# anacarsi/ss25_Hierarchical_Multiscale_Image_Classification

Measured on AMD Instinct MI355X. Metric: 224x224 patches/sec (ResNet18 fwd), higher is better.
Workload: dtype bf16; 1 GPU; resnet18_fwd_880k_patches_bf16; input=uint8 HWC patches resident in HBM, outputs=features[B,512] + logits[B,2] + labels, weights=seeded random init, parallelism=single GPU

## Files before the change

ss25_hierarchical_multiscale_image_classification_amd/csrc/block16_c64.h:

```cpp
#pragma once
#include "halo16.h"

namespace hipac {

typedef __attribute__((ext_vector_type(2))) short s16x2;
__device__ __forceinline__ unsigned relu_pk(unsigned v) {
  return __builtin_bit_cast(unsigned, __builtin_elementwise_max(__builtin_bit_cast(s16x2, v), s16x2{0, 0}));
}

constexpr int kBlkRing = 30;
constexpr int kBlkXPitch = 18 * 128;
constexpr int kBlkIPitch = 16 * 128;
constexpr int kBlkXBytes = 32 * kBlkXPitch + 512;
constexpr int kBlkIBytes = 32 * kBlkIPitch + 256;
constexpr int kBlkRsBytes = 2 * 6144 + 2 * 4096;

#ifndef HIPAC_BLK16_AHEAD
#define HIPAC_BLK16_AHEAD 1
#endif

template <typename T, int NP, int PITCH>
__device__ __forceinline__ void c64_strip16_mfma(const typename Elem<T>::frag (&wreg)[9][2][2], const int (&lb)[NP][3],
                                                 const float* __restrict__ bl, f32x4 (&acc)[2 * NP][2]) {
  using frag = typename Elem<T>::frag;
  constexpr int NR = 2 * NP;
#pragma unroll
  for (int t = 0; t < 2; ++t) {
    const f32x4 b = *reinterpret_cast<const f32x4*>(bl + 16 * t);
#pragma unroll
    for (int i = 0; i < NR; ++i) acc[i][t] = b;
  }
  asm volatile("s_waitcnt lgkmcnt(0)" ::: "memory");
  constexpr int AH = HIPAC_BLK16_AHEAD;
  frag fr[AH + 1][NR];
  auto rd = [&](auto S, auto I) {
    constexpr int s = decltype(S)::value, i = decltype(I)::value;
    constexpr int tap = s >> 1, kk = s & 1, kh = tap / 3, kw = tap % 3;
    lds_read16<((i & 1) + kh) * PITCH>(fr[s % (AH + 1)][i], (unsigned)(lb[i >> 1][kw] ^ (kk << 6)));
  };
  __builtin_amdgcn_s_setprio(1);
  static_for<AH>([&](auto S) { static_for<NR>([&](auto I) { rd(S, I); }); });
  static_for<18>([&](auto S) {
    constexpr int s = decltype(S)::value, tap = s >> 1, kk = s & 1;
    static_for<NR>([&](auto I) {
      constexpr int i = decltype(I)::value;
      if constexpr (s + AH < 18) rd(std::integral_constant<int, s + AH>{}, I);
      constexpr int full = (18 - 1 - s < AH - 1 ? 18 - 1 - s : AH - 1);
      wait_lgkmcnt<(NR - 1 - i) + full * NR + (s + AH < 18 ? i + 1 : 0)>();
      Asm16<T>::mfma(acc[i][0], wreg[tap][kk][0], fr[s % (AH + 1)][i]);
      Asm16<T>::mfma(acc[i][1], wreg[tap][kk][1], fr[s % (AH + 1)][i]);
    });
  });
  __builtin_amdgcn_s_setprio(0);
  asm volatile("s_nop 7\n\ts_nop 7\n\ts_nop 3" ::: "memory");
}

template <typename T>
__global__ __launch_bounds__(512, 2) void block16_c64_kernel(const T* __restrict__ in, const T* __restrict__ w1,
                                                             const float* __restrict__ b1, const T* __restrict__ w2,
                                                             const float* __restrict__ b2, T* __restrict__ out,
                                                             int n_img) {
  using E = Elem<T>;
  using frag = typename E::frag;
  using vec4 = typename E::vec4;
  constexpr int H = 56, W = 56, C = 64, RING = kBlkRing, XP = kBlkXPitch, IP = kBlkIPitch;
  __shared__ __attribute__((aligned(1024))) unsigned char smem[kBlkXBytes + kBlkIBytes + kBlkRsBytes + 512];
  unsigned char* const Xr = smem;
  unsigned char* const Ir = smem + kBlkXBytes;
  float* const Bl = reinterpret_cast<float*>(smem + kBlkXBytes + kBlkIBytes + kBlkRsBytes);

  const int tid = threadIdx.x, lane = tid & 63;
  const int wave = __builtin_amdgcn_readfirstlane(tid >> 6);
  const int team = wave >> 2, tw = wave & 3, nh = tw & 1, mh = tw >> 1;
  const int n16 = lane & 15, g = lane >> 4;
  const int lx = n16 < 4 ? 2 * n16 : (n16 < 12 ? 2 * n16 - 7 : 2 * n16 - 16);
  unsigned char* const Rw = smem + kBlkXBytes + kBlkIBytes + (mh == 0 ? nh * 6144 : 2 * 6144 + nh * 4096);

  if (tid < 64) Bl[tid] = b1[tid];
  else if (tid < 128) Bl[tid] = b2[tid - 64];

  const int xcd = blockIdx.x & 7, slot = blockIdx.x >> 3, nslots = gridDim.x >> 3;
  const int n_x = n_img > xcd ? (n_img - xcd + 7) >> 3 : 0;
  const int nst = 4 * n_x;
  const int ns = nst > slot ? (nst - slot + nslots - 1) / nslots : 0;
  if (ns == 0) return;

  frag wreg[9][2][2];
  {
    const char* wb = reinterpret_cast<const char*>(team ? w2 : w1) + (size_t)(nh * 32 + n16) * (9 * C * 2) + 16 * g;
#pragma unroll
    for (int tap = 0; tap < 9; ++tap)
#pragma unroll
      for (int kk = 0; kk < 2; ++kk)
#pragma unroll
        for (int t = 0; t < 2; ++t) wreg[tap][kk][t] = *reinterpret_cast<const frag*>(wb + t * 16 * (9 * C * 2) + tap * 128 + kk * 64);
  }

  const rsrc_t x_rsrc = make_rsrc(in, n_img * (H * W * C * 2));

  constexpr int NKP = 5;
  int relo[NKP];
#pragma unroll
  for (int kp = 0; kp < NKP; ++kp) {
    const int q = 8 * (tw + 4 * kp) + (lane >> 3);
    const int rr = (q * 3641) >> 16;
    const int j = q - 18 * rr;
    const int c = (lane & 7) ^ ((j >> 1) & 7);
    relo[kp] = (((rr * W + j) << 7) + (c << 4)) | (j < 2 ? 1 : 0) | (j >= 16 ? 2 : 0) | (rr == 0 ? 4 : 0) | (rr >= 1 ? 8 : 0);
  }
  auto x_rows = [&](int img, int x0, int L0, int rb, int np, int rowmask) {
    const int sb = ((img * H + L0 - 1) * W + x0 - 2) << 7;
    const int smask = (x0 == 0 ? 1 : 0) | (x0 == 42 ? 2 : 0) | rowmask;
    static_for<NKP>([&](auto KP) {
      constexpr int kp = decltype(KP)::value;
      const int p = tw + 4 * kp;
      if (p < np) {
        asm volatile("" : "+v"(relo[kp]));
        const int off = (relo[kp] & smask) ? (int)0x80000000 : (relo[kp] & ~15) + sb;
        buffer_load_lds16(x_rsrc, Xr + rb * XP + p * 1024, off, 0);
      }
    });
  };
  auto x_group = [&](int img, int x0, int gq) {
    const int rb = 8 * gq >= RING ? 8 * gq - RING : 8 * gq;
    x_rows(img, x0, 8 * gq, rb, gq == 7 ? 5 : 18, gq == 0 ? 4 : (gq == 7 ? 8 : 0));
    if (gq == 3) x_rows(img, x0, RING, 0, 5, 0);
  };
  auto strip_img = [&](int k) { return (((slot + k * nslots) >> 2) << 3) + xcd; };
  auto strip_x0 = [&](int k) { return ((slot + k * nslots) & 3) * 14; };

  const int lds_base = (int)(unsigned)(size_t)(__attribute__((address_space(3))) unsigned char*)smem;
  int la[3];
#pragma unroll
  for (int kw = 0; kw < 3; ++kw) {
    const int j = lx + kw;
    la[kw] = (j << 7) + (((((j >> 1) & 7)) ^ g) << 4) + (team ? kBlkXBytes : 0) + lds_base;
  }
  const int iw_lane = (lx << 7) + ((g & 1) << 3);
  const int iw_pos = ((nh << 2) + (g >> 1)) ^ ((lx >> 1) & 7);
  const float* const bl = Bl + team * 64 + nh * 32 + 4 * g;

#pragma unroll
  for (int tap = 0; tap < 9; ++tap)
#pragma unroll
    for (int kk = 0; kk < 2; ++kk)
#pragma unroll
      for (int t = 0; t < 2; ++t) asm volatile("" ::"v"(wreg[tap][kk][t]));
  if (team == 0) {
    x_group(strip_img(0), strip_x0(0), 0);
    x_group(strip_img(0), strip_x0(0), 1);
    wait_vmcnt<0>();
  }
  asm volatile("s_waitcnt lgkmcnt(0)" ::: "memory");
  __builtin_amdgcn_s_barrier();

  const int n_steps = 7 * ns;
  f32x4 acc[4][2];
  int pend_n = 0, pend_y = 0;
  const int rs_px = lane >> 2;
  const int rs_off = (((rs_px < 14 ? rs_px : 13)) * C + nh * 32 + 8 * ((lane & 3) ^ ((rs_px >> 2) & 3))) * 2;
  auto fetch_resid = [&](int pix0, int y0, int sl) {
    const int sb = (pix0 + y0 * W) << 7;
#pragma unroll
    for (int rho = 0; rho < 2; ++rho) buffer_load_lds16(x_rsrc, Rw + sl * 2048 + rho * 1024, rs_off + rho * (W * C * 2), sb);
  };
  const int rs_rd = lx * 64 + 8 * (g & 1);
  const int rs_sw = (lx >> 2) & 3;
  const int out_lane = (lx * C + nh * 32 + 16 * (g & 1) + 8 * (g >> 1)) * 2;
  auto epilogue_b = [&](auto A0, int pix0, int y0, int sl) {
    constexpr int a0 = decltype(A0)::value;
#pragma unroll
    for (int rho = 0; rho < 2; ++rho) {
      unsigned P[2][2];
#pragma unroll
      for (int t = 0; t < 2; ++t) {
        const vec4 rv = *reinterpret_cast<const vec4*>(Rw + sl * 2048 + rho * 1024 + rs_rd + (((2 * t + (g >> 1)) ^ rs_sw) << 4));
        const f32x4& a = acc[a0 + rho][t];
        P[t][0] = relu_pk(PackPair<T>::pack_rn(a[0] + (float)rv[0], a[1] + (float)rv[1]));
        P[t][1] = relu_pk(PackPair<T>::pack_rn(a[2] + (float)rv[2], a[3] + (float)rv[3]));
      }
      permlane16_swap(P[0][0], P[1][0]);
      permlane16_swap(P[0][1], P[1][1]);
      char* const dst = reinterpret_cast<char*>(out) + ((size_t)(unsigned)(pix0 + (y0 + rho) * W) << 7) + out_lane;
      if (lx < 14) store16_out(dst, u32x4{P[0][0], P[0][1], P[1][0], P[1][1]});
    }
  };
  int pend_pix = 0, pend_sl = 0;
  auto flush_b = [&]() {
    if (pend_n) {
      wait_vmcnt<0>();
      epilogue_b(std::integral_constant<int, 0>{}, pend_pix, pend_y, pend_sl);
      if (pend_n == 2) epilogue_b(std::integral_constant<int, 2>{}, pend_pix, pend_y + 2, pend_sl + 1);
      pend_n = 0;
    }
  };
  auto step_barrier = [&]() {
    asm volatile("s_waitcnt lgkmcnt(0)" ::: "memory");
    __builtin_amdgcn_s_barrier();
  };
  if (team == 0) {
    for (int G = 0; G <= n_steps; ++G) {
      if (G < n_steps) {
        const int k = G / 7, m = G - 7 * k;
        const int img = strip_img(k), x0 = strip_x0(k);
        if (m <= 4) x_group(img, x0, m + 2);
        else if (m == 5) {
          x_group(img, x0, 7);
          if (k + 1 < ns) x_group(strip_img(k + 1), strip_x0(k + 1), 0);
        } else if (k + 1 < ns) x_group(strip_img(k + 1), strip_x0(k + 1), 1);
        if (m == 0 || m == 6)
          *reinterpret_cast<u32x2*>(Ir + (m == 0 ? 0 : 27) * IP + tw * 512 + lane * 8) = u32x2{0u, 0u};
        const int y0a = 8 * m + 4 * mh;
        int lb[2][3];
#pragma unroll
        for (int p = 0; p < 2; ++p) {
          const int y0 = y0a + 2 * p;
          const int wbase = (y0 >= RING ? y0 - RING : y0) * XP;
#pragma unroll
          for (int kw = 0; kw < 3; ++kw) lb[p][kw] = la[kw] + wbase;
        }
        c64_strip16_mfma<T, 2, XP>(wreg, lb, bl, acc);
        const bool col_ok = !((x0 == 0 && lx == 0) || (x0 == 42 && lx == 15));
#pragma unroll
        for (int i = 0; i < 4; ++i) {
          const int Lr = y0a + i + 1;
          const bool twice = Lr == RING || Lr == RING + 1;
          unsigned char* const dst = Ir + (Lr >= RING ? Lr - RING : Lr) * IP + iw_lane;
          unsigned char* const dst2 = Ir + Lr * IP + iw_lane;
#pragma unroll
          for (int t = 0; t < 2; ++t) {
            u32x2 pk;
            pk[0] = relu_pk(PackPair<T>::pack_rn(acc[i][t][0], acc[i][t][1]));
            pk[1] = relu_pk(PackPair<T>::pack_rn(acc[i][t][2], acc[i][t][3]));
            if (!col_ok) pk = u32x2{0u, 0u};
            *reinterpret_cast<u32x2*>(dst + ((iw_pos ^ (2 * t)) << 4)) = pk;
            if (twice) *reinterpret_cast<u32x2*>(dst2 + ((iw_pos ^ (2 * t)) << 4)) = pk;
          }
        }
      }
      wait_vmcnt<0>();
      step_barrier();
    }
  } else {
    for (int G = 0; G <= n_steps; ++G) {
      flush_b();
      if (G >= 1) {
        const int k = (G - 1) / 7, mp = G - 7 * k;
        int yp = 8 * mp - 10 + 4 * mh, ys = -1;
        bool has_pair = true;
        if (mp == 1) {
          if (mh == 0) yp = 0;
          else has_pair = false, ys = 4;
        } else if (mp == 7) {
          if (mh == 0) yp = 46, ys = 50;
          else yp = 52;
        }
        const int pix0 = strip_img(k) * (H * W) + strip_x0(k);
        if (has_pair) {
          fetch_resid(pix0, yp, 0);
          fetch_resid(pix0, yp + 2, 1);
        }
        if (ys >= 0) fetch_resid(pix0, ys, has_pair ? 2 : 0);
        pend_pix = pix0;
        if (has_pair) {
          int lb[2][3];
#pragma unroll
          for (int p = 0; p < 2; ++p) {
            const int y0 = yp + 2 * p;
            const int wbase = (y0 >= RING ? y0 - RING : y0) * IP;
#pragma unroll
            for (int kw = 0; kw < 3; ++kw) lb[p][kw] = la[kw] + wbase;
          }
          c64_strip16_mfma<T, 2, IP>(wreg, lb, bl, acc);
          pend_n = 2, pend_y = yp, pend_sl = 0;
        }
        if (ys >= 0) {
          flush_b();
          int lb[1][3];
          const int wbase = (ys >= RING ? ys - RING : ys) * IP;
#pragma unroll
          for (int kw = 0; kw < 3; ++kw) lb[0][kw] = la[kw] + wbase;
          f32x4(&acc1)[2][2] = reinterpret_cast<f32x4(&)[2][2]>(acc[0]);
          c64_strip16_mfma<T, 1, IP>(wreg, lb, bl, acc1);
          pend_n = 1, pend_y = ys, pend_sl = has_pair ? 2 : 0;
        }
      }
      step_barrier();
    }
    flush_b();
  }
}

}
```

Before: 312,700 patches/s.

## Read residual from the staged input ring in LDS instead of reloading from HBM

```diff
diff --git a/ss25_hierarchical_multiscale_image_classification_amd/csrc/block16_c64.h b/ss25_hierarchical_multiscale_image_classification_amd/csrc/block16_c64.h
--- a/ss25_hierarchical_multiscale_image_classification_amd/csrc/block16_c64.h
+++ b/ss25_hierarchical_multiscale_image_classification_amd/csrc/block16_c64.h
@@ -9,11 +9,11 @@
 }
 
 constexpr int kBlkRing = 30;
+constexpr int kBlkXRing = 29;
 constexpr int kBlkXPitch = 18 * 128;
 constexpr int kBlkIPitch = 16 * 128;
 constexpr int kBlkXBytes = 32 * kBlkXPitch + 512;
 constexpr int kBlkIBytes = 32 * kBlkIPitch + 256;
-constexpr int kBlkRsBytes = 2 * 6144 + 2 * 4096;
 
 #ifndef HIPAC_BLK16_AHEAD
 #define HIPAC_BLK16_AHEAD 1
@@ -63,18 +63,17 @@
   using E = Elem<T>;
   using frag = typename E::frag;
   using vec4 = typename E::vec4;
-  constexpr int H = 56, W = 56, C = 64, RING = kBlkRing, XP = kBlkXPitch, IP = kBlkIPitch;
-  __shared__ __attribute__((aligned(1024))) unsigned char smem[kBlkXBytes + kBlkIBytes + kBlkRsBytes + 512];
+  constexpr int H = 56, W = 56, C = 64, RING = kBlkRing, XRING = kBlkXRing, XP = kBlkXPitch, IP = kBlkIPitch;
+  __shared__ __attribute__((aligned(1024))) unsigned char smem[kBlkXBytes + kBlkIBytes + 512];
   unsigned char* const Xr = smem;
   unsigned char* const Ir = smem + kBlkXBytes;
-  float* const Bl = reinterpret_cast<float*>(smem + kBlkXBytes + kBlkIBytes + kBlkRsBytes);
+  float* const Bl = reinterpret_cast<float*>(smem + kBlkXBytes + kBlkIBytes);
 
   const int tid = threadIdx.x, lane = tid & 63;
   const int wave = __builtin_amdgcn_readfirstlane(tid >> 6);
   const int team = wave >> 2, tw = wave & 3, nh = tw & 1, mh = tw >> 1;
   const int n16 = lane & 15, g = lane >> 4;
   const int lx = n16 < 4 ? 2 * n16 : (n16 < 12 ? 2 * n16 - 7 : 2 * n16 - 16);
-  unsigned char* const Rw = smem + kBlkXBytes + kBlkIBytes + (mh == 0 ? nh * 6144 : 2 * 6144 + nh * 4096);
 
   if (tid < 64) Bl[tid] = b1[tid];
   else if (tid < 128) Bl[tid] = b2[tid - 64];
@@ -98,7 +97,7 @@
 
   const rsrc_t x_rsrc = make_rsrc(in, n_img * (H * W * C * 2));
 
-  constexpr int NKP = 5;
+  constexpr int NKP = 6;
   int relo[NKP];
 #pragma unroll
   for (int kp = 0; kp < NKP; ++kp) {
@@ -106,26 +105,31 @@
     const int rr = (q * 3641) >> 16;
     const int j = q - 18 * rr;
     const int c = (lane & 7) ^ ((j >> 1) & 7);
-    relo[kp] = (((rr * W + j) << 7) + (c << 4)) | (j < 2 ? 1 : 0) | (j >= 16 ? 2 : 0) | (rr == 0 ? 4 : 0) | (rr >= 1 ? 8 : 0);
-  }
-  auto x_rows = [&](int img, int x0, int L0, int rb, int np, int rowmask) {
+    relo[kp] = (((rr * W + j) << 7) + (c << 4)) | (j < 2 ? 1 : 0) | (j >= 16 ? 2 : 0) | (rr == 0 ? 4 : 0) | (rr == 7 ? 8 : 0);
+  }
+  auto x_rows = [&](int img, int x0, int L0, int rb, int np, int rowmask, int cut) {
     const int sb = ((img * H + L0 - 1) * W + x0 - 2) << 7;
     const int smask = (x0 == 0 ? 1 : 0) | (x0 == 42 ? 2 : 0) | rowmask;
     static_for<NKP>([&](auto KP) {
       constexpr int kp = decltype(KP)::value;
       const int p = tw + 4 * kp;
-      if (p < np) {
+      if (p < np && !(p == cut && lane >= 32)) {
         asm volatile("" : "+v"(relo[kp]));
         const int off = (relo[kp] & smask) ? (int)0x80000000 : (relo[kp] & ~15) + sb;
         buffer_load_lds16(x_rsrc, Xr + rb * XP + p * 1024, off, 0);
       }
     });
   };
-  auto x_group = [&](int img, int x0, int gq) {
-    const int rb = 8 * gq >= RING ? 8 * gq - RING : 8 * gq;
-    x_rows(img, x0, 8 * gq, rb, gq == 7 ? 5 : 18, gq == 0 ? 4 : (gq == 7 ? 8 : 0));
-    if (gq == 3) x_rows(img, x0, RING, 0, 5, 0);
-  };
+  auto x_step = [&](int img, int x0, int m) {
+    if (m == 2) {
+      x_rows(img, x0, 26, 26, 14, 0, -1);
+      x_rows(img, x0, XRING, 0, 12, 0, -1);
+    } else {
+      const int L0 = 8 * m + 10;
+      x_rows(img, x0, L0, L0 >= XRING ? L0 - XRING : L0, 18, m == 5 ? 8 : 0, -1);
+    }
+  };
+  auto x_head = [&](int img, int x0) { x_rows(img, x0, 0, 0, 23, 4, 22); };
   auto strip_img = [&](int k) { return (((slot + k * nslots) >> 2) << 3) + xcd; };
   auto strip_x0 = [&](int k) { return ((slot + k * nslots) & 3) * 14; };
 
@@ -147,8 +151,7 @@
 #pragma unroll
       for (int t = 0; t < 2; ++t) asm volatile("" ::"v"(wreg[tap][kk][t]));
   if (team == 0) {
-    x_group(strip_img(0), strip_x0(0), 0);
-    x_group(strip_img(0), strip_x0(0), 1);
+    x_head(strip_img(0), strip_x0(0));
     wait_vmcnt<0>();
   }
   asm volatile("s_waitcnt lgkmcnt(0)" ::: "memory");
@@ -156,25 +159,19 @@
 
   const int n_steps = 7 * ns;
   f32x4 acc[4][2];
-  int pend_n = 0, pend_y = 0;
-  const int rs_px = lane >> 2;
-  const int rs_off = (((rs_px < 14 ? rs_px : 13)) * C + nh * 32 + 8 * ((lane & 3) ^ ((rs_px >> 2) & 3))) * 2;
-  auto fetch_resid = [&](int pix0, int y0, int sl) {
-    const int sb = (pix0 + y0 * W) << 7;
-#pragma unroll
-    for (int rho = 0; rho < 2; ++rho) buffer_load_lds16(x_rsrc, Rw + sl * 2048 + rho * 1024, rs_off + rho * (W * C * 2), sb);
-  };
-  const int rs_rd = lx * 64 + 8 * (g & 1);
-  const int rs_sw = (lx >> 2) & 3;
+  const int xs_lane = ((lx + 2) << 7) + ((g & 1) << 3);
+  const int xs_pos = ((nh << 2) + (g >> 1)) ^ (((lx + 2) >> 1) & 7);
   const int out_lane = (lx * C + nh * 32 + 16 * (g & 1) + 8 * (g >> 1)) * 2;
-  auto epilogue_b = [&](auto A0, int pix0, int y0, int sl) {
+  auto epilogue_b = [&](auto A0, int pix0, int y0) {
     constexpr int a0 = decltype(A0)::value;
 #pragma unroll
     for (int rho = 0; rho < 2; ++rho) {
       unsigned P[2][2];
+      const int Lx = y0 + rho + 1;
+      const unsigned char* const xr = Xr + (Lx >= XRING ? Lx - XRING : Lx) * XP + xs_lane;
 #pragma unroll
       for (int t = 0; t < 2; ++t) {
-        const vec4 rv = *reinterpret_cast<const vec4*>(Rw + sl * 2048 + rho * 1024 + rs_rd + (((2 * t + (g >> 1)) ^ rs_sw) << 4));
+        const vec4 rv = *reinterpret_cast<const vec4*>(xr + ((xs_pos ^ (2 * t)) << 4));
         const f32x4& a = acc[a0 + rho][t];
         P[t][0] = relu_pk(PackPair<T>::pack_rn(a[0] + (float)rv[0], a[1] + (float)rv[1]));
         P[t][1] = relu_pk(PackPair<T>::pack_rn(a[2] + (float)rv[2], a[3] + (float)rv[3]));
@@ -183,15 +180,6 @@
       permlane16_swap(P[0][1], P[1][1]);
       char* const dst = reinterpret_cast<char*>(out) + ((size_t)(unsigned)(pix0 + (y0 + rho) * W) << 7) + out_lane;
       if (lx < 14) store16_out(dst, u32x4{P[0][0], P[0][1], P[1][0], P[1][1]});
-    }
-  };
-  int pend_pix = 0, pend_sl = 0;
-  auto flush_b = [&]() {
-    if (pend_n) {
-      wait_vmcnt<0>();
-      epilogue_b(std::integral_constant<int, 0>{}, pend_pix, pend_y, pend_sl);
-      if (pend_n == 2) epilogue_b(std::integral_constant<int, 2>{}, pend_pix, pend_y + 2, pend_sl + 1);
-      pend_n = 0;
     }
   };
   auto step_barrier = [&]() {
@@ -203,11 +191,8 @@
       if (G < n_steps) {
         const int k = G / 7, m = G - 7 * k;
         const int img = strip_img(k), x0 = strip_x0(k);
-        if (m <= 4) x_group(img, x0, m + 2);
-        else if (m == 5) {
-          x_group(img, x0, 7);
-          if (k + 1 < ns) x_group(strip_img(k + 1), strip_x0(k + 1), 0);
-        } else if (k + 1 < ns) x_group(strip_img(k + 1), strip_x0(k + 1), 1);
+        if (m <= 5) x_step(img, x0, m);
+        else if (k + 1 < ns) x_head(strip_img(k + 1), strip_x0(k + 1));
         if (m == 0 || m == 6)
           *reinterpret_cast<u32x2*>(Ir + (m == 0 ? 0 : 27) * IP + tw * 512 + lane * 8) = u32x2{0u, 0u};
         const int y0a = 8 * m + 4 * mh;
@@ -215,7 +200,7 @@
 #pragma unroll
         for (int p = 0; p < 2; ++p) {
           const int y0 = y0a + 2 * p;
-          const int wbase = (y0 >= RING ? y0 - RING : y0) * XP;
+          const int wbase = (y0 > XRING ? y0 - XRING : y0) * XP;
 #pragma unroll
           for (int kw = 0; kw < 3; ++kw) lb[p][kw] = la[kw] + wbase;
         }
@@ -243,7 +228,6 @@
     }
   } else {
     for (int G = 0; G <= n_steps; ++G) {
-      flush_b();
       if (G >= 1) {
         const int k = (G - 1) / 7, mp = G - 7 * k;
         int yp = 8 * mp - 10 + 4 * mh, ys = -1;
@@ -257,12 +241,6 @@
         }
         const int pix0 = strip_img(k) * (H * W) + strip_x0(k);
         if (has_pair) {
-          fetch_resid(pix0, yp, 0);
-          fetch_resid(pix0, yp + 2, 1);
-        }
-        if (ys >= 0) fetch_resid(pix0, ys, has_pair ? 2 : 0);
-        pend_pix = pix0;
-        if (has_pair) {
           int lb[2][3];
 #pragma unroll
           for (int p = 0; p < 2; ++p) {
@@ -272,23 +250,22 @@
             for (int kw = 0; kw < 3; ++kw) lb[p][kw] = la[kw] + wbase;
           }
           c64_strip16_mfma<T, 2, IP>(wreg, lb, bl, acc);
-          pend_n = 2, pend_y = yp, pend_sl = 0;
+          epilogue_b(std::integral_constant<int, 0>{}, pix0, yp);
+          epilogue_b(std::integral_constant<int, 2>{}, pix0, yp + 2);
         }
         if (ys >= 0) {
-          flush_b();
           int lb[1][3];
           const int wbase = (ys >= RING ? ys - RING : ys) * IP;
 #pragma unroll
           for (int kw = 0; kw < 3; ++kw) lb[0][kw] = la[kw] + wbase;
           f32x4(&acc1)[2][2] = reinterpret_cast<f32x4(&)[2][2]>(acc[0]);
           c64_strip16_mfma<T, 1, IP>(wreg, lb, bl, acc1);
-          pend_n = 1, pend_y = ys, pend_sl = has_pair ? 2 : 0;
+          epilogue_b(std::integral_constant<int, 0>{}, pix0, ys);
         }
       }
       step_barrier();
     }
-    flush_b();
-  }
-}
-
-}
+  }
+}
+
+}
```

Measured after the change: 314,700 patches/s (median of 6 runs). Within noise of the previous version (+0.7%).
